# dariopagliaricci/Metal-PathTracer-arm64

Measured on AMD Instinct MI355X. Metric: Msamples/sec (whole node) at 1920×1080, depth 8; PFM RMSE vs Embree ref, higher is better.
Workload: dtype f32; 1 GPU; BASELINE configs[1]: Cornell box + one 70,688-triangle OBJ mesh, 1920x1080, depth 8, 256 spp, seed 1337; partition=8-row bands round-robin over 1 rank(s), RCCL gather of the HDR buffer

## Files before the change

metal-pathtracer-arm64_amd/csrc/kernels/traverse.h:

```cpp
#pragma once

#include "device_types.h"
#include "vec.h"

namespace ptrk {

struct TraceCounters {
    uint32_t nodes;
    uint32_t prims;
    uint32_t waveNodeSteps = 0, wavePrimSteps = 0, leaves = 0;
};

typedef __attribute__((address_space(3))) uint32_t LdsWord;

struct LaneStack {
    LdsWord* lds;
    uint32_t* spill;
    uint32_t spillStride;
    uint32_t limit;
    uint32_t sp;
    __device__ __forceinline__ uint32_t* spillSlot(uint32_t level) const {
        const uint32_t column = blockIdx.x * kTraceBlock + threadIdx.x;
        return spill + static_cast<size_t>(level - kLdsStackLevels) * spillStride + column;
    }
    __device__ __forceinline__ void push(uint32_t v) {
        if (sp < kLdsStackLevels) {
            lds[sp * kTraceBlock] = v;
        } else if (sp < limit) {
            *spillSlot(sp) = v;
        } else {
            return;
        }
        ++sp;
    }
    __device__ __forceinline__ uint32_t pop() {
        --sp;
        return (sp < kLdsStackLevels) ? lds[sp * kTraceBlock] : *spillSlot(sp);
    }
};

typedef uint32_t u32x4 __attribute__((ext_vector_type(4)));

struct SceneMem {
    __amdgpu_buffer_rsrc_t nodes;
    __amdgpu_buffer_rsrc_t tris;
    __amdgpu_buffer_rsrc_t wide;
};

__device__ __forceinline__ SceneMem sceneMem(const SceneView& sc) {
    SceneMem m;
    const void* nodes = sc.useQuantized ? static_cast<const void*>(sc.qnodes) : static_cast<const void*>(sc.nodes);
    m.nodes = __builtin_amdgcn_make_buffer_rsrc(const_cast<void*>(nodes), 0, sc.nodeBytes, 0x00020000);
    m.tris = __builtin_amdgcn_make_buffer_rsrc(const_cast<float4*>(sc.tris), 0, sc.triBytes, 0x00020000);
    m.wide = __builtin_amdgcn_make_buffer_rsrc(const_cast<uint4*>(sc.wnodes), 0, sc.wideBytes, 0x00020000);
    return m;
}

__device__ __forceinline__ uint4 load16u(__amdgpu_buffer_rsrc_t r, uint32_t byteOffset) {
    const u32x4 v = __builtin_amdgcn_raw_buffer_load_b128(r, byteOffset, 0, 0);
    return make_uint4(v.x, v.y, v.z, v.w);
}
__device__ __forceinline__ float4 load16f(__amdgpu_buffer_rsrc_t r, uint32_t byteOffset) {
    const u32x4 v = __builtin_amdgcn_raw_buffer_load_b128(r, byteOffset, 0, 0);
    return make_float4(__uint_as_float(v.x), __uint_as_float(v.y), __uint_as_float(v.z), __uint_as_float(v.w));
}

struct TraceHit {
    float t;
    uint32_t prim;
};

typedef float v2f __attribute__((ext_vector_type(2)));

__device__ __forceinline__ bool slabTest(f3 lo, f3 hi, f3 oi, f3 inv, float tnear, float tfar, float& entry) {
    const v2f tx = __builtin_elementwise_fma((v2f){lo.x, hi.x}, (v2f){inv.x, inv.x}, (v2f){-oi.x, -oi.x});
    const v2f ty = __builtin_elementwise_fma((v2f){lo.y, hi.y}, (v2f){inv.y, inv.y}, (v2f){-oi.y, -oi.y});
    const v2f tz = __builtin_elementwise_fma((v2f){lo.z, hi.z}, (v2f){inv.z, inv.z}, (v2f){-oi.z, -oi.z});
    const float ax = tx.x, bx = tx.y, ay = ty.x, by = ty.y, az = tz.x, bz = tz.y;
    const float t0 = fmaxf(fmaxf(fminf(ax, bx), fminf(ay, by)), fmaxf(fminf(az, bz), tnear));
    const float t1 = fminf(fminf(fmaxf(ax, bx), fmaxf(ay, by)), fminf(fmaxf(az, bz), tfar));
    entry = t0;
    return t0 <= t1 * 1.0000004f;
}

__device__ __forceinline__ bool slabTestOrdered(f3 nearQ, f3 farQ, f3 oi, f3 inv, float tnear, float tfar, float& entry) {
    const v2f tx = __builtin_elementwise_fma((v2f){nearQ.x, farQ.x}, (v2f){inv.x, inv.x}, (v2f){-oi.x, -oi.x});
    const v2f ty = __builtin_elementwise_fma((v2f){nearQ.y, farQ.y}, (v2f){inv.y, inv.y}, (v2f){-oi.y, -oi.y});
    const v2f tz = __builtin_elementwise_fma((v2f){nearQ.z, farQ.z}, (v2f){inv.z, inv.z}, (v2f){-oi.z, -oi.z});
    const float t0 = fmaxf(fmaxf(tx.x, ty.x), fmaxf(tz.x, tnear));
    const float t1 = fminf(fminf(tx.y, ty.y), fminf(tz.y, tfar));
    entry = t0;
    return t0 <= t1 * 1.0000004f;
}

__device__ __forceinline__ bool triangleTest(f3 v0, f3 e1, f3 e2, f3 org, f3 dir, float tnear, float tfar,
                                             float& t, float& u, float& v) {
    const f3 Ng = cross(e2, e1);
    const f3 C = v0 - org;
    const f3 R = cross(C, dir);
    const float den = dot(Ng, dir);
    const float absDen = fabsf(den);
    const float sgn = signbit(den) ? -1.0f : 1.0f;
    const float U = dot(R, e2) * sgn;
    const float V = dot(R, e1) * sgn;
    if (!(den != 0.0f && U >= 0.0f && V >= 0.0f && (U + V) <= absDen)) return false;
    const float T = dot(Ng, C) * sgn;
    if (!(absDen * tnear < T && T <= absDen * tfar)) return false;
    const float rcpAbsDen = 1.0f / absDen;
    t = T * rcpAbsDen;
    u = U * rcpAbsDen;
    v = V * rcpAbsDen;
    return true;
}

__device__ __forceinline__ void triangleUv(f3 v0, f3 e1, f3 e2, f3 org, f3 dir, float& u, float& v) {
    const f3 Ng = cross(e2, e1);
    const f3 C = v0 - org;
    const f3 R = cross(C, dir);
    const float den = dot(Ng, dir);
    const float absDen = fabsf(den);
    const float sgn = signbit(den) ? -1.0f : 1.0f;
    const float U = dot(R, e2) * sgn;
    const float V = dot(R, e1) * sgn;
    const float rcpAbsDen = 1.0f / absDen;
    u = U * rcpAbsDen;
    v = V * rcpAbsDen;
}

__device__ __forceinline__ bool sphereTest(float4 s, f3 org, f3 dir, float tnear, float tfar, float& t) {
    const float rd2 = 1.0f / dot(dir, dir);
    const f3 c0 = mk3(s) - org;
    const float projC0 = dot(c0, dir) * rd2;
    const f3 perp = c0 - projC0 * dir;
    const float l2 = dot(perp, perp);
    const float r2 = s.w * s.w;
    if (!(l2 <= r2)) return false;
    const float td = sqrtf((r2 - l2) * rd2);
    const float tFront = projC0 - td;
    const float tBack = projC0 + td;
    const bool validFront = (tnear <= tFront) && (tFront <= tfar);
    const bool validBack = (tnear <= tBack) && (tBack <= tfar);
    if (!validFront && !validBack) return false;
    t = validFront ? tFront : tBack;
    return true;
}

struct Trav {
    f3 org, dir, inv;
    f3 oi;
    uint32_t selX, selY, selZ;
    float tnear;
    TraceHit hit;
    uint32_t cur;
    uint32_t leafPos;
    bool anyHit;
};

template <int NODES = -1>
__device__ __forceinline__ bool travBegin(const SceneView& sc, Trav& t, f3 org, f3 dir, float tnear, float tfar, bool anyHit,
                                          LaneStack& stack) {
    t.org = org;
    t.dir = dir;
    constexpr float kInvMax = 1.0e28f;
    t.inv = mk3(fminf(fmaxf(__builtin_amdgcn_rcpf(dir.x), -kInvMax), kInvMax), fminf(fmaxf(__builtin_amdgcn_rcpf(dir.y), -kInvMax), kInvMax),
                fminf(fmaxf(__builtin_amdgcn_rcpf(dir.z), -kInvMax), kInvMax));
    if (NODES >= 1 || (NODES < 0 && sc.useQuantized)) {
        const f3 cell = mk3(sc.gridCell[0], sc.gridCell[1], sc.gridCell[2]);
        const f3 invCell = mk3(sc.gridInvCell[0], sc.gridInvCell[1], sc.gridInvCell[2]);
        const f3 orgQ = (org - mk3(sc.gridOrigin[0], sc.gridOrigin[1], sc.gridOrigin[2])) * invCell;
        t.inv = t.inv * cell;
        t.oi = orgQ * t.inv;
    } else {
        t.oi = org * t.inv;
    }
    t.selX = t.inv.x < 0.0f ? 0x01000706u : 0x07060100u;
    t.selY = t.inv.y < 0.0f ? 0x03020504u : 0x05040302u;
    t.selZ = t.inv.z < 0.0f ? 0x01000706u : 0x07060100u;
    t.tnear = tnear;
    t.hit.t = tfar;
    t.hit.prim = kHitMiss;
    t.anyHit = anyHit;
    t.cur = sc.rootRef;
    t.leafPos = 0u;
    stack.sp = 0;
    if (sc.oversizeRef != kRefEmpty) {
        if (sc.rootRef != kRefEmpty) stack.push(sc.rootRef);
        t.cur = sc.oversizeRef;
        return true;
    }
    return sc.rootRef != kRefEmpty;
}

__device__ __forceinline__ bool travAtLeaf(const Trav& t) { return (t.cur & kRefLeafBit) != 0u; }
__device__ __forceinline__ bool travPop(Trav& t, LaneStack& stack) {
    if (stack.sp == 0) return false;
    t.cur = stack.pop();
    t.leafPos = 0u;
    return true;
}

__device__ __forceinline__ f3 gridLo(uint32_t w0, uint32_t w1) {
    return mk3(static_cast<float>(w0 & 0xFFFFu), static_cast<float>(w0 >> 16), static_cast<float>(w1 & 0xFFFFu));
}
__device__ __forceinline__ f3 gridHi(uint32_t w1, uint32_t w2) {
    return mk3(static_cast<float>(w1 >> 16), static_cast<float>(w2 & 0xFFFFu), static_cast<float>(w2 >> 16));
}

template <bool COUNT>
__device__ __forceinline__ bool travWideStep(const SceneMem& mem, Trav& t, LaneStack& stack, TraceCounters& cnt) {
    const uint32_t at = t.cur * 64u;
    const uint4 c0 = load16u(mem.wide, at), c1 = load16u(mem.wide, at + 16u), c2 = load16u(mem.wide, at + 32u), c3 = load16u(mem.wide, at + 48u);
    float k0, k1, k2, k3;
    auto boxTest = [&](const uint4& c, float& k) {
        const uint32_t wx = __builtin_amdgcn_perm(c.y, c.x, t.selX), wy = __builtin_amdgcn_perm(c.z, c.x, t.selY), wz = __builtin_amdgcn_perm(c.z, c.y, t.selZ);
        const f3 nearQ = mk3(static_cast<float>(wx & 0xFFFFu), static_cast<float>(wy & 0xFFFFu), static_cast<float>(wz & 0xFFFFu));
        const f3 farQ = mk3(static_cast<float>(wx >> 16), static_cast<float>(wy >> 16), static_cast<float>(wz >> 16));
        return slabTestOrdered(nearQ, farQ, t.oi, t.inv, t.tnear, t.hit.t, k);
    };
    const bool h0 = boxTest(c0, k0), h1 = boxTest(c1, k1), h2 = boxTest(c2, k2), h3 = boxTest(c3, k3);
    k0 = h0 ? k0 : INFINITY;
    k1 = h1 ? k1 : INFINITY;
    k2 = h2 ? k2 : INFINITY;
    k3 = h3 ? k3 : INFINITY;
    uint32_t r0 = c0.w, r1 = c1.w, r2 = c2.w, r3 = c3.w;
    if (COUNT) ++cnt.nodes;
    t.leafPos = 0u;
    auto exchange = [](float& ka, uint32_t& ra, float& kb, uint32_t& rb) {
        const bool swap = kb < ka;
        const float kLo = swap ? kb : ka, kHi = swap ? ka : kb;
        const uint32_t rLo = swap ? rb : ra, rHi = swap ? ra : rb;
        ka = kLo;
        kb = kHi;
        ra = rLo;
        rb = rHi;
    };
    exchange(k0, r0, k1, r1);
    exchange(k2, r2, k3, r3);
    exchange(k0, r0, k2, r2);
    exchange(k1, r1, k3, r3);
    exchange(k1, r1, k2, r2);
    if (k3 < INFINITY) stack.push(r3);
    if (k2 < INFINITY) stack.push(r2);
    if (k1 < INFINITY) stack.push(r1);
    if (k0 < INFINITY) {
        t.cur = r0;
        return true;
    }
    return travPop(t, stack);
}

template <bool COUNT, int NODES = -1>
__device__ __forceinline__ bool travNodeStep(const SceneView& sc, const SceneMem& mem, Trav& t, LaneStack& stack, TraceCounters& cnt) {
    if (NODES == 2) return travWideStep<COUNT>(mem, t, stack, cnt);
    uint32_t ref0, ref1;
    float e0, e1;
    bool h0, h1;
    if (NODES == 1 || (NODES < 0 && sc.useQuantized)) {
        const uint4 q0 = load16u(mem.nodes, t.cur * 32u), q1 = load16u(mem.nodes, t.cur * 32u + 16u);
        ref0 = q0.w;
        ref1 = q1.w;
        h0 = slabTest(gridLo(q0.x, q0.y), gridHi(q0.y, q0.z), t.oi, t.inv, t.tnear, t.hit.t, e0);
        h1 = slabTest(gridLo(q1.x, q1.y), gridHi(q1.y, q1.z), t.oi, t.inv, t.tnear, t.hit.t, e1);
    } else {
        const uint32_t at = t.cur * 64u;
        const float4 n0 = load16f(mem.nodes, at), n1 = load16f(mem.nodes, at + 16u), n2 = load16f(mem.nodes, at + 32u),
                     n3 = load16f(mem.nodes, at + 48u);
        ref0 = __float_as_uint(n0.w);
        ref1 = __float_as_uint(n1.w);
        h0 = slabTest(mk3(n0), mk3(n1), t.oi, t.inv, t.tnear, t.hit.t, e0);
        h1 = slabTest(mk3(n2), mk3(n3), t.oi, t.inv, t.tnear, t.hit.t, e1);
    }
    h0 = h0 & (ref0 != kRefEmpty);
    h1 = h1 & (ref1 != kRefEmpty);
    if (COUNT) ++cnt.nodes;
    const bool firstIs0 = e0 <= e1;
    const uint32_t nearRef = (h0 & (firstIs0 | !h1)) ? ref0 : ref1;
    const uint32_t farRef = firstIs0 ? ref1 : ref0;
    t.leafPos = 0u;
    if (h0 & h1) stack.push(farRef);
    if (h0 | h1) {
        t.cur = nearRef;
        return true;
    }
    return travPop(t, stack);
}

template <bool COUNT>
__device__ __forceinline__ bool travPrimStep(const SceneView& sc, const SceneMem& mem, Trav& t, LaneStack& stack, TraceCounters& cnt) {
    const uint32_t cur = t.cur;
    const uint32_t first = cur & kRefOffsetMask;
    const uint32_t count = ((cur >> kRefCountShift) & 0xFu) + 1u;
    const uint32_t index = first + t.leafPos;
    if (COUNT) { ++cnt.prims; if (t.leafPos == 0u) { ++cnt.nodes; ++cnt.leaves; } }
    if (cur & kRefSphereBit) {
        float tt;
        if (sphereTest(sc.spheres[index], t.org, t.dir, t.tnear, t.hit.t, tt)) {
            t.hit.t = tt;
            t.hit.prim = index | kHitSphereBit;
            if (t.anyHit) return false;
        }
    } else {
        const uint32_t at = index * 48u;
        const float4 a = load16f(mem.tris, at), b = load16f(mem.tris, at + 16u), c = load16f(mem.tris, at + 32u);
        float tt, u, v;
        if (triangleTest(mk3(a), mk3(b), mk3(c), t.org, t.dir, t.tnear, t.hit.t, tt, u, v) && !(t.anyHit && __float_as_uint(b.w) == t.hit.prim)) {
            t.hit.t = tt;
            t.hit.prim = index;
            if (t.anyHit) return false;
        }
    }
    if (++t.leafPos < count) return true;
    return travPop(t, stack);
}

#ifndef PTR_EXTRA_NODE_STEPS
#define PTR_EXTRA_NODE_STEPS 3
#endif
#ifndef PTR_EXTRA_PRIM_STEPS
#define PTR_EXTRA_PRIM_STEPS 1
#endif
#ifndef PTR_PRIM_BIAS
#define PTR_PRIM_BIAS 2
#endif
#ifndef PTR_REPEAT_NUM
#define PTR_REPEAT_NUM 1
#define PTR_REPEAT_DEN 2
#endif

template <bool COUNT, int NODES = -1>
__device__ __forceinline__ bool travVote(const SceneView& sc, const SceneMem& mem, Trav& t, bool active, LaneStack& stack,
                                         TraceCounters& cnt) {
    const bool wantsPrim = active && travAtLeaf(t);
    const bool wantsNode = active && !travAtLeaf(t);
    const int nPrim = __popcll(__ballot(wantsPrim));
    const int nNode = __popcll(__ballot(wantsNode));
    bool more = true;
    if (nNode >= nPrim * PTR_PRIM_BIAS) {
        if (COUNT) ++cnt.waveNodeSteps;
// ... 38 lines not shown
```

metal-pathtracer-arm64_amd/csrc/kernels/wavefront.hip:

```cpp
#include <hip/hip_runtime.h>

#include <algorithm>

#include "bsdf.h"
#include "device_types.h"
#include "launch.h"
#include <type_traits>
#include "traverse.h"
#include "texture.h"
#include "vec.h"

namespace ptrk {

namespace {

constexpr float kEps = 1.0e-4f;
constexpr float kSpecNeePdfFloor = 1.0e-4f;
constexpr float kSpecNeeInvPdfClamp = 1.0e4f;
constexpr float kMisMin = 1.0e-4f;
constexpr float kMisMax = 0.9999f;
#ifndef PTR_SHADE_BLOCK
#define PTR_SHADE_BLOCK 128
#endif
constexpr uint32_t kShadeBlock = PTR_SHADE_BLOCK;
// ... 308 lines not shown
        const uint32_t idx = prim & ~kHitSphereBit;
        const float4 sp = sc.spheres[idx];
        const uint2 info = sc.sphereInfo[idx];
        const f3 n = normalize(s.position - mk3(sp));
        s.normal = n;
        s.hitShadingNormal = n;
        s.frontFace = dot(dir, n) < 0.0f;
        s.twoSided = true;
        s.primType = 1u;
        s.geomIndex = 0u;
        s.primIndex = info.x;
        s.material = info.y;
        return s;
    }
    const uint32_t triOffset = prim * 48u;
    const float4* tp = byteOffset(sc.tris, triOffset);
    const float4* np = byteOffset(sc.triNormals, triOffset);
    const float4 a = tp[0], b = tp[1], c = tp[2];
    const float4 n0 = np[0], n1 = np[1], n2 = np[2];
    asm volatile("" ::"v"(a.x), "v"(b.x), "v"(c.x), "v"(n0.x), "v"(n1.x), "v"(n2.x));
    const f3 ng = cross(mk3(c), mk3(b));
    if (dot(ng, ng) > 0.0f) s.normal = normalize(ng);
    s.frontFace = dot(dir, s.normal) < 0.0f;
    const f3 adjusted = s.frontFace ? s.normal : -s.normal;
    f3 shading = adjusted;
    const uint32_t meta = __float_as_uint(b.w);
    s.material = __float_as_uint(a.w);
    s.geomIndex = 0u;
    if ((meta >> 30) == 0u) {
        s.primType = 0u;
        s.primIndex = __float_as_uint(c.w);
        s.geomIndex = meta & kTriGeomMask;
        float u, v;
        triangleUv(mk3(a), mk3(b), mk3(c), org, dir, u, v);
        s.bu = u;
        s.bv = v;
        const float w = 1.0f - u - v;
        const f3 interp = (w * mk3(n0) + u * mk3(n1)) + v * mk3(n2);
        if (dot(interp, interp) > 0.0f) {
            shading = normalize(interp);
            if (dot(shading, adjusted) < 0.0f) shading = -shading;
        }
    } else {
        s.primType = 2u;
        s.primIndex = meta & kTriGeomMask;
        shading = mk3(n0);
        if (dot(shading, adjusted) < 0.0f) shading = -shading;
        s.twoSided = __float_as_uint(sc.rects[static_cast<size_t>(s.primIndex) * 5u + 4u].y) != 0u;
    }
    s.hitShadingNormal = shading;
    return s;
}

struct OffsetFrame {
    f3 position, n;
    float distance;
};
__device__ __forceinline__ OffsetFrame offsetFrame(const Surface& s) {
    OffsetFrame of;
    f3 n = s.hitShadingNormal;
    if (dot(n, n) <= 0.0f) n = s.normal;
    if (dot(n, n) <= 0.0f) n = mk3(0.0f, 1.0f, 0.0f);
    of.n = normalize(n);
    of.distance = smax(fabsf(s.t) * 1.0e-4f, kEps);
    of.position = s.position;
    return of;
}
// ... 28 lines not shown
    if (distSq <= 0.0f) return 0.0f;
    const float distance = sqrtf(distSq);
    const f3 direction = toLight / distance;
    float cosLight = dot(-direction, mk3(r[3]));
    if (__float_as_uint(r[4].y) != 0u) {
        cosLight = fabsf(cosLight);
    } else if (cosLight <= 0.0f) {
        return 0.0f;
    }
    if (cosLight <= 0.0f) return 0.0f;
    const float pdfArea = 1.0f / area;
    const float pdfDir = pdfArea * distSq / smax(cosLight, 1.0e-6f);
    return pdfDir * (1.0f / static_cast<float>(sc.rectLightCount));
}

__device__ __forceinline__ bool rectLightHit(const SceneView& sc, const Surface& s, f3 origin, float emissionScale, f3& emission, float& pdf) {
    if (sc.rectLightCount == 0u || sc.rectCount == 0u) return false;
    if (s.primType != 2u || s.primIndex >= sc.rectCount) return false;
    const int32_t li = sc.lightIndexByRect[s.primIndex];
    if (li < 0) return false;
    const float4* L = sc.rectLights + static_cast<size_t>(li) * kRectLightVec4;
    const bool twoSided = L[1].w != 0.0f;
    if (!s.frontFace && !twoSided) return false;
    emission = mk3(L[4]) * emissionScale;
    if (!(dot(emission, emission) > 0.0f)) return false;
    pdf = rectLightPdfForHit(sc, s.primType, s.primIndex, s.position, origin);
    return (pdf > 0.0f) && isfinite(pdf);
}


__device__ __forceinline__ bool nearestRectLight(const SceneView& sc, f3 org, f3 dir, float& tHit, uint32_t& light, uint32_t& half) {
    float best = INFINITY;
    bool found = false;
    for (uint32_t li = 0; li < sc.rectLightCount; ++li) {
        const float4* T = sc.rectLights + static_cast<size_t>(li) * kRectLightVec4 + 5u;
#pragma unroll
        for (uint32_t h = 0; h < 2u; ++h) {
            float tt, tu, tv;
            if (triangleTest(mk3(T[h * 3u]), mk3(T[h * 3u + 1u]), mk3(T[h * 3u + 2u]), org, dir, kEps, best, tt, tu, tv)) {
                best = tt;
                light = li;
                half = h;
                found = true;
            }
        }
    }
    tHit = best;
    return found;
}

__device__ __forceinline__ Surface rectLightSurface(const SceneView& sc, f3 org, f3 dir, float t, uint32_t light, uint32_t half, uint32_t& metaWord) {
    const float4* T = sc.rectLights + static_cast<size_t>(light) * kRectLightVec4 + 5u + half * 3u;
    const float4 b = T[1], c = T[2];
    Surface s;
    s.t = t;
    s.prim = 0u;
    s.bu = 0.0f;
    s.bv = 0.0f;
    s.position = org + t * dir;
    s.normal = mk3(0.0f, 1.0f, 0.0f);
    const f3 ng = cross(mk3(c), mk3(b));
    if (dot(ng, ng) > 0.0f) s.normal = normalize(ng);
    s.hitShadingNormal = s.normal;
    s.frontFace = dot(dir, s.normal) < 0.0f;
    s.twoSided = false;
    metaWord = __float_as_uint(b.w);
    s.primType = 2u;
    s.primIndex = metaWord & kTriGeomMask;
    s.geomIndex = 0u;
    s.material = 0u;
    return s;
}
// ... 61 lines not shown
    if constexpr (COUNT) {
        addCounter(counters, kCntShadowRays, raysAny);
        addCounter(counters, kCntShadowNodes, any.nodes);
        addCounter(counters, kCntShadowPrims, any.prims);
        addCounter(counters, kCntExtendRays, raysClosest);
        addCounter(counters, kCntExtendNodes, closest.nodes);
        addCounter(counters, kCntExtendPrims, closest.prims);
    }
}

}

__global__ void __launch_bounds__(256) k_generate(RenderParams rp, PathPool pool) {
    const uint32_t slot = blockIdx.x * blockDim.x + threadIdx.x;
    if (slot >= pool.slots) return;
    uint32_t flags = 0u, rng = 0u;
    f3 o = mk3(0.0f), d = mk3(0.0f);
    if (slot < rp.itemCount && rp.maxDepth > 0u) {
        beginItem(rp, pool, slot, rng, o, d);
        flags = kFlagAlive | kFlagLastDelta;
    }
    pool.ray0[slot] = mk4(o, d.x);
    pool.ray1[slot] = make_float4(d.y, d.z, 1.0f, __uint_as_float(flags));
    pool.thr[slot] = make_float4(1.0f, 1.0f, 1.0f, __uint_as_float(rng));
    pool.accum[slot] = make_float4(0.0f, 0.0f, 0.0f, __uint_as_float(slot));
    if (pool.signature) pool.signature[slot] = 0u;
    if (pool.cone) pool.cone[slot] = primaryCone(rp);
}

#ifndef PTR_TRAV_WAVES
#define PTR_TRAV_WAVES 8
#endif
#define PTR_EXTEND_ATTR __attribute__((amdgpu_waves_per_eu(PTR_TRAV_WAVES, PTR_TRAV_WAVES)))
template <bool COUNT, bool ALIVE, int NODES>
__global__ void __launch_bounds__(kTraceBlock) PTR_EXTEND_ATTR k_extend(SceneView sc, PathPool pool, uint32_t* spill, uint32_t spillStride, uint32_t* workCounter,
                                                         int kRefillBelow, uint32_t feederChunk, uint32_t* aliveOut) {
    __shared__ uint32_t ldsStack[kLdsStackLevels * kTraceBlock];
    LaneStack stack = laneStack(ldsStack, spill, spillStride, sc);
    TraceCounters cnt{0u, 0u};
    uint32_t rays = 0u;
    uint32_t aliveSeen = 0u;
    uint32_t refills = 0u;
    uint32_t refillCycles = 0u;
    uint32_t activeLanes = 0u, leafLanes = 0u, voteIterations = 0u;
    const long long kernelStart = COUNT ? clock64() : 0ll;

    SceneMem mem = sceneMem(sc);
    bool listed = ALIVE && pool.busyIn != nullptr;
    SubLists lists{0u, pool.slots};
    if (listed) {
        lists.init(pool.busyCountIn, pool.connectRegion);
        if (static_cast<uint64_t>(lists.total) * PTR_BUSY_EXTEND_DIV >= pool.slots) {
            listed = false;
            lists.total = pool.slots;
        }
    }
    WaveFeeder feeder;
    const uint32_t listChunk = shortListChunk(lists.total, (gridDim.x * blockDim.x) >> 6);
    feeder.init(workCounter, lists.total, listed ? listChunk : feederChunk);
    Trav t;
    t.cur = 0u;
    bool active = false;
    uint32_t mySlot = 0u;
    while (true) {
        const int nActive = __popcll(__ballot(active));
        if (nActive < kRefillBelow && !feeder.exhausted) {
            if (COUNT) ++refills;
            const long long refillStart = COUNT ? clock64() : 0ll;
            uint32_t idx = feeder.take(!active);
            if (listed) {
                const uint32_t entry = pool.busyIn[lists.position(idx != WaveFeeder::kNone ? idx : 0u, pool.connectRegion)];
                if (idx != WaveFeeder::kNone) idx = (entry & kBusyAliveBit) ? (entry & ~kBusyAliveBit) : WaveFeeder::kNone;
            }
            const uint32_t at = idx != WaveFeeder::kNone ? idx : 0u;
            const float4 r0 = pool.ray0[at], r1 = pool.ray1[at];
            const bool live = idx != WaveFeeder::kNone && (__float_as_uint(r1.w) & kFlagAlive);
            if (ALIVE) aliveSeen += static_cast<uint32_t>(__popcll(__ballot(live)));
            if (live) {
                mySlot = idx;
                if (COUNT) ++rays;
                active = travBegin<NODES>(sc, t, mk3(r0), mk3(r0.w, r1.x, r1.y), kEps, INFINITY, false, stack);
                if (!active) pool.hit[idx] = make_float2(INFINITY, __uint_as_float(kHitMiss));
            }
            if (COUNT) {
                asm volatile("" ::"v"(t.inv.x), "v"(t.oi.x));
                refillCycles += static_cast<uint32_t>(clock64() - refillStart);
            }
            continue;
        }
        if (nActive == 0) break;
        if (COUNT) {
            activeLanes += static_cast<uint32_t>(nActive);
            leafLanes += static_cast<uint32_t>(__popcll(__ballot(active && travAtLeaf(t))));
            ++voteIterations;
        }
        if (!travVote<COUNT, NODES>(sc, mem, t, active, stack, cnt)) {
            active = false;
            pool.hit[mySlot] = make_float2(t.hit.t, __uint_as_float(t.hit.prim));
        }
    }
    if (ALIVE) {
        if (laneId() == 0 && aliveSeen != 0u) atomicAdd(aliveOut, aliveSeen);
    }
    if (COUNT) {
        addCounter(pool.counters, kCntExtendRays, rays);
        addCounter(pool.counters, kCntExtendNodes, cnt.nodes);
        addCounter(pool.counters, kCntExtendPrims, cnt.prims);
        addCounter(pool.counters, kCntExtendLeaves, cnt.leaves);
        addCounter(pool.counters, kCntExtendWaveNodeSteps, cnt.waveNodeSteps);
        addCounter(pool.counters, kCntExtendWavePrimSteps, cnt.wavePrimSteps);
        addCounter(pool.counters, kCntExtendRefillPasses, refills);
        addCounter(pool.counters, kCntExtendActiveLanes, activeLanes >> 6);
        addCounter(pool.counters, kCntExtendLeafLanes, leafLanes >> 6);
        addCounter(pool.counters, kCntExtendVoteIterations, voteIterations);
        addCounter(pool.counters, kCntExtendRefillTicks, refillCycles >> 4);
        addCounter(pool.counters, kCntExtendWaveTicks, static_cast<uint32_t>((clock64() - kernelStart) >> 4));
    }
}
// ... 379 lines not shown
    const UniformRows Lu = uniformRows(sc.rectLights);
    auto row = [&](uint32_t i) { return ONE ? Lu[i] : Lv[i]; };
    const float4 l0 = row(0), l1 = row(1), l2 = row(2), l3 = row(3);
    const f3 samplePoint = (mk3(l0) + lu * mk3(l1)) + lv * mk3(l2);
    const f3 toLight = samplePoint - sf.position;
    const float distSq = dot(toLight, toLight);
    if (!(distSq > 0.0f && l0.w > 0.0f)) return false;
    const float distance = sqrtf(distSq);
    const f3 ldir = toLight / distance;
    float cosLight = dot(-ldir, mk3(l3));
    if (l1.w != 0.0f) cosLight = fabsf(cosLight);
    if (!(cosLight > 0.0f)) return false;
    const float pdfArea = 1.0f / l0.w;
    const float pdfDir = pdfArea * distSq / smax(cosLight, 1.0e-6f);
    const float pdf = pdfDir * (1.0f / static_cast<float>(nL));
    const f3 emission = mk3(row(4)) * rp.emissionScale;
    const float nDotL = smax(dot(n, ldir), 0.0f);
    if (!(pdf > 0.0f && isfinite(pdf) && (dot(emission, emission) > 0.0f) && nDotL > 0.0f)) return false;
    if (COUNT) counts.stage[4] += 1u;
    const BsdfEvalResult be = evalBsdf<SSS, MATS>(mat, sf.position, n, wo, ldir, cc);
    if (!neeContributes<SSS>(be, cc)) return false;
    const float w = neeWeight<SSS>(pdf, be.pdf, cc);
    f3 contrib = (emission * be.value) * nDotL;
    contrib *= w / pdf;
    if (!finite3(contrib)) return false;
    const f3 clamped = clampFirefly(thr, contrib, cc);
    if (!(clamped.x > 0.0f || clamped.y > 0.0f || clamped.z > 0.0f)) return false;
    const float shadowMax = smax(distance * (1.0f - rp.shadowSlack) - kEps, kEps);
    const f3 shadowOrg = offsetOrigin(of, ldir);
    float tt, tu, tv;
    bool occludedByLight = false;
    if (COUNT) counts.stage[5] += 1u;
    if (l3.w != 0.0f) {
        occludedByLight = triangleTest(mk3(row(5)), mk3(row(6)), mk3(row(7)), shadowOrg, ldir, kEps, shadowMax, tt, tu, tv) ||
                          triangleTest(mk3(row(8)), mk3(row(9)), mk3(row(10)), shadowOrg, ldir, kEps, shadowMax, tt, tu, tv);
    }
    if (occludedByLight) return false;
    if (COUNT) counts.stage[6] += 1u;
    storeRecord(pool, slot, 0u, 0u, shadowOrg, shadowMax, ldir, clamped, static_cast<float>(depth), mk3(0.0f));
    return true;
}

template <bool SSS>
__device__ __forceinline__ bool surfaceIsDelta(const Mat& mat, uint32_t type, const ClampCfg& cc) {
    bool surfaceDelta = materialIsDelta(mat);
    if (SSS && cc.metalPbr && type == 7u) surfaceDelta = mat.roughness01() <= 1.0e-3f;
    return surfaceDelta;
}

constexpr int kShadeDense = 0, kShadeListed = 1, kShadeTail = 2;
template <bool COUNT, bool SSS, bool TEX, int MODE, uint32_t MATS = kAllMaterials>
__device__ __forceinline__ void shadeSlot(const RenderParams& rp, const SceneView& sc, const PathPool& pool, const uint32_t slot, const bool inRange,
                                          const bool drained, const uint32_t listWave, ShadeCounts& counts, const EnvLodView& env) {
    constexpr bool TAIL = MODE == kShadeTail;
    const long long tLoad = partBegin<COUNT>();
    const uint32_t at = inRange ? slot : 0u;
    float4 ray1v = pool.ray1[at];
    if (!TAIL && drained) {
        const uint32_t peek = __float_as_uint(ray1v.w);
        const bool busy = inRange && (peek & (kFlagAlive | kFlagFlush | (kFlagPendingMask << kFlagPendingShift))) != 0u;
        if (__ballot(busy) == 0ull) return;
    }
    const float4 ray0v = pool.ray0[at];
    uint2 reservation = make_uint2(0u, 0u);
    if (MODE == kShadeDense && (slot & ~63u) < pool.slots) reservation = pool.itemReserve[__builtin_amdgcn_readfirstlane(slot / 64u)];
    const float2 hitv = pool.hit[at];
    const float4 thr4 = pool.thr[at];
    const float4 acc4 = pool.accum[at];
// ... 590 lines not shown
    f3 result = mk3(0.0f);
    if (COUNT) ++raysClosest;
    const TraceHit h = traverse<false, COUNT>(sc, org, dir, kEps, INFINITY, stack, cntClosest);
    if (h.prim == kHitMiss || sc.materialCount == 0u) return result;
    const Surface cs = reconstruct(sc, org, dir, h.t, h.prim);
    f3 tmpE;
    float tmpP;
    if (sc.rectLightCount > 0u && rectLightHit(sc, cs, org, rp.emissionScale, tmpE, tmpP)) return result;
    const Mat cm{sc.materials + static_cast<size_t>(min(cs.material, sc.materialCount - 1u)) * kMaterialVec4};
    if (!materialIsDelta(cm)) return result;
    f3 cn = cs.normal;
    if (dot(cn, cn) <= 0.0f) cn = mk3(0.0f, 1.0f, 0.0f);
    cn = normalize(cn);
    const f3 cin = normalize(dir);
    const BsdfSampleResult s2 = sampleBsdf(cm, cs.position, cn, -cin, cin, cs.frontFace, rngCopy, cc);
    if (!(s2.pdf > 0.0f && s2.isDelta && dot(s2.dir, s2.dir) > 0.0f && finite3(s2.weight))) return result;
    const f3 d2 = normalize(s2.dir);
    const f3 o2 = offsetOrigin(cs, d2);
    const f3 w2 = weight * s2.weight;
    const float pdf2 = bsdfPdf * s2.pdf;
    if (sc.envSampling) {
        if (COUNT) ++raysAny;
        result += alongEnv<COUNT>(rp, sc, cc, o2, d2, w2, pdf2, thr, stack, cntAny);
    }
    if (sc.rectLightCount > 0u) {
        if (COUNT) ++raysClosest;
        result += alongRect<COUNT>(rp, sc, cc, o2, d2, w2, pdf2, thr, stack, cntClosest);
    }
    return result;
}

}

template <bool COUNT, int NODES>
__global__ void __launch_bounds__(kTraceBlock) PTR_EXTEND_ATTR k_connect(RenderParams rp, SceneView sc, PathPool pool, uint32_t* spill, uint32_t spillStride,
                                                          uint32_t* workCounter, int kRefillBelow, uint32_t feederChunk) {
    __shared__ uint32_t ldsStack[kLdsStackLevels * kTraceBlock];
    LaneStack stack = laneStack(ldsStack, spill, spillStride, sc);
    TraceCounters cnt{0u, 0u}, cntClosest{0u, 0u};
    uint32_t rays = 0u, raysClosest = 0u, early = 0u;
    const ClampCfg cc = clampCfg(rp);

    SceneMem mem = sceneMem(sc);
    SubLists lists;
    lists.init(pool.connectCount, pool.connectRegion);
    WaveFeeder feeder;
    feeder.init(workCounter, lists.total, shortListChunk(lists.total, (gridDim.x * blockDim.x) >> 6));
    Trav t;
    t.cur = 0u;
    bool active = false;
    uint32_t mySlot = 0u, bits = 0u;
    float4* const recBase = pool.rec[0].org;
    const uint32_t slots = pool.recStride;
    uint32_t myRecAt = 0u;
    while (true) {
        const int nActive = __popcll(__ballot(active));
        const bool idleBits = __ballot(!active && bits != 0u) != 0ull;
        if (nActive < kRefillBelow && (idleBits || !feeder.exhausted)) {
            if (!feeder.exhausted) {
                const uint32_t idx = feeder.take(!active && bits == 0u);
                const uint32_t at = lists.position(idx != WaveFeeder::kNone ? idx : 0u, pool.connectRegion);
                if (idx != WaveFeeder::kNone) {
                    const uint32_t entry = pool.connectList[at];
                    mySlot = entry & ((1u << kConnectMaskShift) - 1u);
                    bits = entry >> kConnectMaskShift;
                }
            }
            if (!active && bits != 0u) {
                const uint32_t rec = static_cast<uint32_t>(__ffs(static_cast<int>(bits))) - 1u;
                bits &= bits - 1u;
                myRecAt = rec * 4u * slots + mySlot;
                const float4 o4 = recBase[myRecAt], d4 = recBase[myRecAt + slots];
                const uint32_t kind = __float_as_uint(d4.w);
                if (kind != 2u) {
                    const bool any = kind != 1u;
                    if (COUNT) { if (any) ++rays; else ++raysClosest; }
                    active = travBegin<NODES>(sc, t, mk3(o4), mk3(d4), kEps, any ? o4.w : INFINITY, any, stack);
                    if (kind == 3u) t.hit.prim = __float_as_uint(recBase[myRecAt + 3u * slots].x);
                    if (!active && kind == 1u) recBase[myRecAt + 2u * slots] = make_float4(0.0f, 0.0f, 0.0f, 0.0f);
                }
            }
            continue;
        }
        if (nActive == 0) break;
        {
            TraceCounters step{0u, 0u};
            const bool more = travVote<COUNT, NODES>(sc, mem, t, active, stack, step);
            if (COUNT) {
                TraceCounters& dst = t.anyHit ? cnt : cntClosest;
                dst.nodes += step.nodes;
                dst.prims += step.prims;
            }
            if (!more) {
                active = false;
                float4* const a = recBase + myRecAt + 2u * slots;
                if (t.anyHit) {
                    if (COUNT) early += anyHitFound(t.hit.prim) ? 1u : 0u;
                    if (anyHitFound(t.hit.prim)) *a = make_float4(0.0f, 0.0f, 0.0f, 0.0f);
                } else {
                    const float4 a4 = *a;
                    const f3 c = rectContribution(rp, sc, cc, t.org, t.dir, t.hit, mk3(a4), a4.w, mk3(recBase[myRecAt + 3u * slots]));
                    *a = mk4(c, 0.0f);
                }
            }
        }
    }
    addTraceCounters<COUNT>(pool.counters, rays, cnt, raysClosest, cntClosest);
    if (COUNT) addCounter(pool.counters, kCntShadowEarlyExit, early);
}

template <bool COUNT>
__global__ void __launch_bounds__(kTraceBlock) k_connect_chain(RenderParams rp, SceneView sc, PathPool pool, uint32_t* spill, uint32_t spillStride) {
    __shared__ uint32_t ldsStack[kLdsStackLevels * kTraceBlock];
    const uint32_t gtid = blockIdx.x * kTraceBlock + threadIdx.x;
    LaneStack stack = laneStack(ldsStack, spill, spillStride, sc);
    TraceCounters cnt{0u, 0u}, cntClosest{0u, 0u};
    uint32_t rays = 0u, raysClosest = 0u;
    const ClampCfg cc = clampCfg(rp);
    for (uint32_t slot = gtid; slot < pool.slots; slot += gridDim.x * kTraceBlock) {
        if (!((__float_as_uint(pool.ray1[slot].w) >> kFlagPendingShift) & (1u << 4))) continue;
        const ShadowRecordView& r = pool.rec[4];
        const float4 d4 = r.dir[slot];
        if (__float_as_uint(d4.w) != 2u) continue;
        const float4 o4 = r.org[slot], a4 = r.a[slot];
        const f3 c = mneeChain<COUNT>(rp, sc, cc, mk3(o4), mk3(d4), __float_as_uint(o4.w), mk3(a4), a4.w, mk3(r.b[slot]), stack, cnt,
                                      cntClosest, rays, raysClosest);
        r.a[slot] = mk4(c, 0.0f);
    }
    addTraceCounters<COUNT>(pool.counters, rays, cnt, raysClosest, cntClosest);
}

__global__ void __launch_bounds__(256) k_tail_collect(PathPool pool, uint32_t* list, uint32_t* listCount) {
    __shared__ uint32_t found[4][64];
    const uint32_t wave = threadIdx.x >> 6, lane = laneId();
// ... 156 lines not shown
            f3 sn = sf.hitShadingNormal;
            if (dot(sn, sn) <= 0.0f) sn = sf.normal;
            if (mat.type() == 2u) sn = sf.normal;
            sn = normalize(sn);
            a = mk4(mat.baseColor(), 1.0f);
            n = mk4(sn * 0.5f + mk3(0.5f), h.t);
        }
        albedo[pixel] = a;
        normal[pixel] = n;
    }
}

__device__ __forceinline__ PtrHit ptrHitOf(const SceneView& sc, f3 org, f3 dir, const TraceHit& h, bool anyHit) {
    float hu = 0.0f, hv = 0.0f;
    PtrHit r;
    r.t = -1.0f;
    r.u = 0.0f;
    r.v = 0.0f;
    r.primType = 0u;
    r.geomIndex = 0u;
    r.primIndex = 0u;
    r.ng[0] = r.ng[1] = r.ng[2] = 0.0f;
    r.pad = 0u;
    if (h.prim != kHitMiss) {
        r.t = anyHit ? 0.0f : h.t;
        if (!anyHit) {
            if (h.prim & kHitSphereBit) {
                r.primType = 1u;
                r.primIndex = sc.sphereInfo[h.prim & kHitIndexMask].x;
            } else {
                const float4* tp = sc.tris + static_cast<size_t>(h.prim & kHitIndexMask) * 3u;
                const float4 t0 = tp[0], t1 = tp[1], t2 = tp[2];
                const uint32_t meta = __float_as_uint(t1.w);
                triangleUv(mk3(t0), mk3(t1), mk3(t2), org, dir, hu, hv);
                r.u = hu;
                r.v = hv;
                const f3 ng = cross(mk3(t2), mk3(t1));
                r.ng[0] = ng.x;
                r.ng[1] = ng.y;
                r.ng[2] = ng.z;
                if ((meta >> 30) == 0u) {
                    r.primType = 0u;
                    r.geomIndex = meta & kTriGeomMask;
                    r.primIndex = __float_as_uint(t2.w);
                } else {
                    r.primType = 2u;
                    r.primIndex = meta & kTriGeomMask;
                }
            }
        }
    }
    return r;
}

template <bool ANY>
__global__ void __launch_bounds__(kTraceBlock) k_trace_rays(SceneView sc, const float4* rays, uint64_t n, PtrHit* out, uint32_t* spill,
                                                             uint32_t spillStride, uint64_t* counters) {
    __shared__ uint32_t ldsStack[kLdsStackLevels * kTraceBlock];
    const uint32_t gtid = blockIdx.x * kTraceBlock + threadIdx.x;
    LaneStack stack = laneStack(ldsStack, spill, spillStride, sc);
    TraceCounters cnt{0u, 0u};
    for (uint64_t i = gtid; i < n; i += static_cast<uint64_t>(gridDim.x) * kTraceBlock) {
        const float4 a = rays[i * 2u], b = rays[i * 2u + 1u];
        const f3 org = mk3(a), dir = mk3(b);
        const TraceHit h = traverse<ANY, true>(sc, org, dir, a.w, b.w, stack, cnt);
        out[i] = ptrHitOf(sc, org, dir, h, ANY);
    }
// ... 488 lines not shown
```

Before: 2529 Msamples/s.

## Pack ray/triangle math into paired f32 ops and reload cold kernel args

Rewrites the triangle test and slab test so the ray and triangle data are held as float pairs, letting the compiler use packed v_pk_* f32 FMA/add/mul and inline-asm cross blends. The ray state now stores origin/direction pairs and precomputed (inv, -oi) slab pairs instead of separate org/dir/inv/oi vectors. Cold scene and render params in k_extend and k_connect are re-read from the kernarg segment through an opaque pointer, so they are not kept live in registers across the traversal loop. The aim is fewer VALU instructions and lower register pressure in the traversal kernels. In exchange it relies on inline asm and compiler behaviour, and could change rounding slightly.

```diff
diff --git a/metal-pathtracer-arm64_amd/csrc/kernels/traverse.h b/metal-pathtracer-arm64_amd/csrc/kernels/traverse.h
--- a/metal-pathtracer-arm64_amd/csrc/kernels/traverse.h
+++ b/metal-pathtracer-arm64_amd/csrc/kernels/traverse.h
@@ -40,6 +40,7 @@
 };
 
 typedef uint32_t u32x4 __attribute__((ext_vector_type(4)));
+typedef float v4f __attribute__((ext_vector_type(4)));
 
 struct SceneMem {
     __amdgpu_buffer_rsrc_t nodes;
@@ -60,6 +61,9 @@
     const u32x4 v = __builtin_amdgcn_raw_buffer_load_b128(r, byteOffset, 0, 0);
     return make_uint4(v.x, v.y, v.z, v.w);
 }
+__device__ __forceinline__ v4f load16v(__amdgpu_buffer_rsrc_t r, uint32_t byteOffset) {
+    return __builtin_bit_cast(v4f, __builtin_amdgcn_raw_buffer_load_b128(r, byteOffset, 0, 0));
+}
 __device__ __forceinline__ float4 load16f(__amdgpu_buffer_rsrc_t r, uint32_t byteOffset) {
     const u32x4 v = __builtin_amdgcn_raw_buffer_load_b128(r, byteOffset, 0, 0);
     return make_float4(__uint_as_float(v.x), __uint_as_float(v.y), __uint_as_float(v.z), __uint_as_float(v.w));
@@ -72,39 +76,123 @@
 
 typedef float v2f __attribute__((ext_vector_type(2)));
 
-__device__ __forceinline__ bool slabTest(f3 lo, f3 hi, f3 oi, f3 inv, float tnear, float tfar, float& entry) {
-    const v2f tx = __builtin_elementwise_fma((v2f){lo.x, hi.x}, (v2f){inv.x, inv.x}, (v2f){-oi.x, -oi.x});
-    const v2f ty = __builtin_elementwise_fma((v2f){lo.y, hi.y}, (v2f){inv.y, inv.y}, (v2f){-oi.y, -oi.y});
-    const v2f tz = __builtin_elementwise_fma((v2f){lo.z, hi.z}, (v2f){inv.z, inv.z}, (v2f){-oi.z, -oi.z});
+struct SlabAxes {
+    v2f x, y, z;
+};
+
+__device__ __forceinline__ v2f slabPlanes(float p0, float p1, v2f axis) {
+    return __builtin_elementwise_fma((v2f){p0, p1}, __builtin_shufflevector(axis, axis, 0, 0), __builtin_shufflevector(axis, axis, 1, 1));
+}
+
+__device__ __forceinline__ float minWithTfar(float a, float tfar) {
+    float r;
+    asm("v_min_f32 %0, %1, %2" : "=v"(r) : "v"(a), "v"(tfar));
+    return r;
+}
+
+__device__ __forceinline__ bool slabTest(f3 lo, f3 hi, const SlabAxes& ax3, float tnear, float tfar, float& entry) {
+    const v2f tx = slabPlanes(lo.x, hi.x, ax3.x), ty = slabPlanes(lo.y, hi.y, ax3.y), tz = slabPlanes(lo.z, hi.z, ax3.z);
     const float ax = tx.x, bx = tx.y, ay = ty.x, by = ty.y, az = tz.x, bz = tz.y;
     const float t0 = fmaxf(fmaxf(fminf(ax, bx), fminf(ay, by)), fmaxf(fminf(az, bz), tnear));
-    const float t1 = fminf(fminf(fmaxf(ax, bx), fmaxf(ay, by)), fminf(fmaxf(az, bz), tfar));
+    const float t1 = fminf(fminf(fmaxf(ax, bx), fmaxf(ay, by)), minWithTfar(fmaxf(az, bz), tfar));
     entry = t0;
     return t0 <= t1 * 1.0000004f;
 }
 
-__device__ __forceinline__ bool slabTestOrdered(f3 nearQ, f3 farQ, f3 oi, f3 inv, float tnear, float tfar, float& entry) {
-    const v2f tx = __builtin_elementwise_fma((v2f){nearQ.x, farQ.x}, (v2f){inv.x, inv.x}, (v2f){-oi.x, -oi.x});
-    const v2f ty = __builtin_elementwise_fma((v2f){nearQ.y, farQ.y}, (v2f){inv.y, inv.y}, (v2f){-oi.y, -oi.y});
-    const v2f tz = __builtin_elementwise_fma((v2f){nearQ.z, farQ.z}, (v2f){inv.z, inv.z}, (v2f){-oi.z, -oi.z});
+__device__ __forceinline__ bool slabTestOrdered(f3 nearQ, f3 farQ, const SlabAxes& ax3, float tnear, float tfar, float& entry) {
+    const v2f tx = slabPlanes(nearQ.x, farQ.x, ax3.x), ty = slabPlanes(nearQ.y, farQ.y, ax3.y), tz = slabPlanes(nearQ.z, farQ.z, ax3.z);
     const float t0 = fmaxf(fmaxf(tx.x, ty.x), fmaxf(tz.x, tnear));
-    const float t1 = fminf(fminf(tx.y, ty.y), fminf(tz.y, tfar));
+    const float t1 = fminf(fminf(tx.y, ty.y), minWithTfar(tz.y, tfar));
     entry = t0;
     return t0 <= t1 * 1.0000004f;
 }
 
-__device__ __forceinline__ bool triangleTest(f3 v0, f3 e1, f3 e2, f3 org, f3 dir, float tnear, float tfar,
-                                             float& t, float& u, float& v) {
-    const f3 Ng = cross(e2, e1);
-    const f3 C = v0 - org;
-    const f3 R = cross(C, dir);
-    const float den = dot(Ng, dir);
-    const float absDen = fabsf(den);
-    const float sgn = signbit(den) ? -1.0f : 1.0f;
-    const float U = dot(R, e2) * sgn;
-    const float V = dot(R, e1) * sgn;
-    if (!(den != 0.0f && U >= 0.0f && V >= 0.0f && (U + V) <= absDen)) return false;
-    const float T = dot(Ng, C) * sgn;
+struct s2f {
+    float x, y;
+};
+__device__ __forceinline__ s2f operator*(s2f a, s2f b) { return s2f{a.x * b.x, a.y * b.y}; }
+__device__ __forceinline__ s2f operator-(s2f a, s2f b) { return s2f{a.x - b.x, a.y - b.y}; }
+
+template <int LO, int HI> __device__ __forceinline__ v2f pick(v2f p) { return __builtin_shufflevector(p, p, LO, HI); }
+template <int LO, int HI> __device__ __forceinline__ s2f pick(s2f p) { return s2f{LO ? p.y : p.x, HI ? p.y : p.x}; }
+__device__ __forceinline__ v2f crossBlend(v2f m1, v2f m2) {
+    v2f xy;
+    asm("v_pk_add_f32 %0, %1, %2 neg_lo:[0,1] neg_hi:[1,0]" : "=v"(xy) : "v"(m1), "v"(m2));
+    return xy;
+}
+__device__ __forceinline__ s2f crossBlend(s2f m1, s2f m2) { return s2f{m1.x - m2.x, m2.y - m1.y}; }
+__device__ __forceinline__ float sumHalves(v2f p) {
+    float r;
+    asm("v_add_f32 %0, %1, %2" : "=v"(r) : "v"(p.x), "v"(p.y));
+    return r;
+}
+__device__ __forceinline__ float sumHalves(s2f p) { return p.x + p.y; }
+
+template <typename P>
+struct RayPairsT {
+    P orgXY, dirXY, orgZdirZ;
+};
+typedef RayPairsT<v2f> RayPairs;
+template <typename P = v2f>
+__device__ __forceinline__ RayPairsT<P> rayPairs(f3 org, f3 dir) { return RayPairsT<P>{P{org.x, org.y}, P{dir.x, dir.y}, P{org.z, dir.z}}; }
+__device__ __forceinline__ f3 rayOrg(const RayPairs& r) { return mk3(r.orgXY.x, r.orgXY.y, r.orgZdirZ.x); }
+__device__ __forceinline__ f3 rayDir(const RayPairs& r) { return mk3(r.dirXY.x, r.dirXY.y, r.orgZdirZ.y); }
+
+template <typename P>
+struct TrianglePairsT {
+    P v0XY, v0Z_, e1XY, e1Z_, e2XY, e2Z_;
+};
+__device__ __forceinline__ TrianglePairsT<v2f> trianglePairs(v4f a, v4f b, v4f c) { return TrianglePairsT<v2f>{a.xy, a.zw, b.xy, b.zw, c.xy, c.zw}; }
+__device__ __forceinline__ TrianglePairsT<v2f> trianglePairs(const float4& a, const float4& b, const float4& c) {
+    return TrianglePairsT<v2f>{(v2f){a.x, a.y}, (v2f){a.z, a.w}, (v2f){b.x, b.y}, (v2f){b.z, b.w}, (v2f){c.x, c.y}, (v2f){c.z, c.w}};
+}
+__device__ __forceinline__ TrianglePairsT<s2f> triangleScalars(const float4& a, const float4& b, const float4& c) {
+    return TrianglePairsT<s2f>{s2f{a.x, a.y}, s2f{a.z, a.z}, s2f{b.x, b.y}, s2f{b.z, b.z}, s2f{c.x, c.y}, s2f{c.z, c.z}};
+}
+
+template <int AZ, int BZ, typename P>
+__device__ __forceinline__ P crossPairs(P aXY, P aZ_, P bXY, P bZ_, float& z) {
+    const P bYX = pick<1, 0>(bXY);
+    const P m1 = pick<1, 0>(aXY) * pick<BZ, BZ>(bZ_);
+    const P m2 = pick<AZ, AZ>(aZ_) * bYX;
+    const P m3 = aXY * bYX;
+    z = m3.x - m3.y;
+    return crossBlend(m1, m2);
+}
+template <typename P>
+__device__ __forceinline__ float dotPairs(P aXY, float aZ, P bXY, float bZ) {
+    const P m = aXY * bXY;
+    return (m.x + m.y) + aZ * bZ;
+}
+
+template <typename P>
+struct TriangleTermsT {
+    P ngXY, cXY, uv;
+    float ngZ, cZ, den, sgn;
+};
+template <typename P>
+__device__ __forceinline__ TriangleTermsT<P> triangleTerms(const TrianglePairsT<P>& tri, const RayPairsT<P>& ray) {
+    TriangleTermsT<P> k;
+    float rZ;
+    k.ngXY = crossPairs<0, 0>(tri.e2XY, tri.e2Z_, tri.e1XY, tri.e1Z_, k.ngZ);
+    k.cXY = tri.v0XY - ray.orgXY;
+    const P cZ_ = tri.v0Z_ - ray.orgZdirZ;
+    k.cZ = cZ_.x;
+    const float dirZ = ray.orgZdirZ.y;
+    const P rXY = crossPairs<0, 1>(k.cXY, cZ_, ray.dirXY, ray.orgZdirZ, rZ);
+    k.den = dotPairs(k.ngXY, k.ngZ, ray.dirXY, dirZ);
+    k.sgn = signbit(k.den) ? -1.0f : 1.0f;
+    k.uv = P{dotPairs(rXY, rZ, tri.e2XY, tri.e2Z_.x), dotPairs(rXY, rZ, tri.e1XY, tri.e1Z_.x)} * P{k.sgn, k.sgn};
+    return k;
+}
+
+template <typename P>
+__device__ __forceinline__ bool triangleTest(const TrianglePairsT<P>& tri, const RayPairsT<P>& ray, float tnear, float tfar, float& t, float& u, float& v) {
+    const TriangleTermsT<P> k = triangleTerms(tri, ray);
+    const float absDen = fabsf(k.den);
+    const float U = k.uv.x, V = k.uv.y;
+    if (!(k.den != 0.0f && U >= 0.0f && V >= 0.0f && sumHalves(k.uv) <= absDen)) return false;
+    const float T = dotPairs(k.ngXY, k.ngZ, k.cXY, k.cZ) * k.sgn;
     if (!(absDen * tnear < T && T <= absDen * tfar)) return false;
     const float rcpAbsDen = 1.0f / absDen;
     t = T * rcpAbsDen;
@@ -113,18 +201,12 @@
     return true;
 }
 
-__device__ __forceinline__ void triangleUv(f3 v0, f3 e1, f3 e2, f3 org, f3 dir, float& u, float& v) {
-    const f3 Ng = cross(e2, e1);
-    const f3 C = v0 - org;
-    const f3 R = cross(C, dir);
-    const float den = dot(Ng, dir);
-    const float absDen = fabsf(den);
-    const float sgn = signbit(den) ? -1.0f : 1.0f;
-    const float U = dot(R, e2) * sgn;
-    const float V = dot(R, e1) * sgn;
-    const float rcpAbsDen = 1.0f / absDen;
-    u = U * rcpAbsDen;
-    v = V * rcpAbsDen;
+template <typename P>
+__device__ __forceinline__ void triangleUv(const TrianglePairsT<P>& tri, const RayPairsT<P>& ray, float& u, float& v) {
+    const TriangleTermsT<P> k = triangleTerms(tri, ray);
+    const float rcpAbsDen = 1.0f / fabsf(k.den);
+    u = k.uv.x * rcpAbsDen;
+    v = k.uv.y * rcpAbsDen;
 }
 
 __device__ __forceinline__ bool sphereTest(float4 s, f3 org, f3 dir, float tnear, float tfar, float& t) {
@@ -146,8 +228,8 @@
 }
 
 struct Trav {
-    f3 org, dir, inv;
-    f3 oi;
+    RayPairs ray;
+    SlabAxes slab;
     uint32_t selX, selY, selZ;
     float tnear;
     TraceHit hit;
@@ -159,23 +241,24 @@
 template <int NODES = -1>
 __device__ __forceinline__ bool travBegin(const SceneView& sc, Trav& t, f3 org, f3 dir, float tnear, float tfar, bool anyHit,
                                           LaneStack& stack) {
-    t.org = org;
-    t.dir = dir;
+    t.ray = rayPairs(org, dir);
     constexpr float kInvMax = 1.0e28f;
-    t.inv = mk3(fminf(fmaxf(__builtin_amdgcn_rcpf(dir.x), -kInvMax), kInvMax), fminf(fmaxf(__builtin_amdgcn_rcpf(dir.y), -kInvMax), kInvMax),
-                fminf(fmaxf(__builtin_amdgcn_rcpf(dir.z), -kInvMax), kInvMax));
+    f3 inv = mk3(fminf(fmaxf(__builtin_amdgcn_rcpf(dir.x), -kInvMax), kInvMax), fminf(fmaxf(__builtin_amdgcn_rcpf(dir.y), -kInvMax), kInvMax),
+                 fminf(fmaxf(__builtin_amdgcn_rcpf(dir.z), -kInvMax), kInvMax));
+    f3 oi;
     if (NODES >= 1 || (NODES < 0 && sc.useQuantized)) {
         const f3 cell = mk3(sc.gridCell[0], sc.gridCell[1], sc.gridCell[2]);
         const f3 invCell = mk3(sc.gridInvCell[0], sc.gridInvCell[1], sc.gridInvCell[2]);
         const f3 orgQ = (org - mk3(sc.gridOrigin[0], sc.gridOrigin[1], sc.gridOrigin[2])) * invCell;
-        t.inv = t.inv * cell;
-        t.oi = orgQ * t.inv;
+        inv = inv * cell;
+        oi = orgQ * inv;
     } else {
-        t.oi = org * t.inv;
-    }
-    t.selX = t.inv.x < 0.0f ? 0x01000706u : 0x07060100u;
-    t.selY = t.inv.y < 0.0f ? 0x03020504u : 0x05040302u;
-    t.selZ = t.inv.z < 0.0f ? 0x01000706u : 0x07060100u;
+        oi = org * inv;
+    }
+    t.slab = SlabAxes{(v2f){inv.x, -oi.x}, (v2f){inv.y, -oi.y}, (v2f){inv.z, -oi.z}};
+    t.selX = inv.x < 0.0f ? 0x01000706u : 0x07060100u;
+    t.selY = inv.y < 0.0f ? 0x03020504u : 0x05040302u;
+    t.selZ = inv.z < 0.0f ? 0x01000706u : 0x07060100u;
     t.tnear = tnear;
     t.hit.t = tfar;
     t.hit.prim = kHitMiss;
@@ -215,7 +298,7 @@
         const uint32_t wx = __builtin_amdgcn_perm(c.y, c.x, t.selX), wy = __builtin_amdgcn_perm(c.z, c.x, t.selY), wz = __builtin_amdgcn_perm(c.z, c.y, t.selZ);
         const f3 nearQ = mk3(static_cast<float>(wx & 0xFFFFu), static_cast<float>(wy & 0xFFFFu), static_cast<float>(wz & 0xFFFFu));
         const f3 farQ = mk3(static_cast<float>(wx >> 16), static_cast<float>(wy >> 16), static_cast<float>(wz >> 16));
-        return slabTestOrdered(nearQ, farQ, t.oi, t.inv, t.tnear, t.hit.t, k);
+        return slabTestOrdered(nearQ, farQ, t.slab, t.tnear, t.hit.t, k);
     };
     const bool h0 = boxTest(c0, k0), h1 = boxTest(c1, k1), h2 = boxTest(c2, k2), h3 = boxTest(c3, k3);
     k0 = h0 ? k0 : INFINITY;
@@ -259,16 +342,16 @@
         const uint4 q0 = load16u(mem.nodes, t.cur * 32u), q1 = load16u(mem.nodes, t.cur * 32u + 16u);
         ref0 = q0.w;
         ref1 = q1.w;
-        h0 = slabTest(gridLo(q0.x, q0.y), gridHi(q0.y, q0.z), t.oi, t.inv, t.tnear, t.hit.t, e0);
-        h1 = slabTest(gridLo(q1.x, q1.y), gridHi(q1.y, q1.z), t.oi, t.inv, t.tnear, t.hit.t, e1);
+        h0 = slabTest(gridLo(q0.x, q0.y), gridHi(q0.y, q0.z), t.slab, t.tnear, t.hit.t, e0);
+        h1 = slabTest(gridLo(q1.x, q1.y), gridHi(q1.y, q1.z), t.slab, t.tnear, t.hit.t, e1);
     } else {
         const uint32_t at = t.cur * 64u;
         const float4 n0 = load16f(mem.nodes, at), n1 = load16f(mem.nodes, at + 16u), n2 = load16f(mem.nodes, at + 32u),
                      n3 = load16f(mem.nodes, at + 48u);
         ref0 = __float_as_uint(n0.w);
         ref1 = __float_as_uint(n1.w);
-        h0 = slabTest(mk3(n0), mk3(n1), t.oi, t.inv, t.tnear, t.hit.t, e0);
-        h1 = slabTest(mk3(n2), mk3(n3), t.oi, t.inv, t.tnear, t.hit.t, e1);
+        h0 = slabTest(mk3(n0), mk3(n1), t.slab, t.tnear, t.hit.t, e0);
+        h1 = slabTest(mk3(n2), mk3(n3), t.slab, t.tnear, t.hit.t, e1);
     }
     h0 = h0 & (ref0 != kRefEmpty);
     h1 = h1 & (ref1 != kRefEmpty);
@@ -294,16 +377,18 @@
     if (COUNT) { ++cnt.prims; if (t.leafPos == 0u) { ++cnt.nodes; ++cnt.leaves; } }
     if (cur & kRefSphereBit) {
         float tt;
-        if (sphereTest(sc.spheres[index], t.org, t.dir, t.tnear, t.hit.t, tt)) {
+        if (sphereTest(sc.spheres[index], rayOrg(t.ray), rayDir(t.ray), t.tnear, t.hit.t, tt)) {
             t.hit.t = tt;
             t.hit.prim = index | kHitSphereBit;
             if (t.anyHit) return false;
         }
     } else {
         const uint32_t at = index * 48u;
-        const float4 a = load16f(mem.tris, at), b = load16f(mem.tris, at + 16u), c = load16f(mem.tris, at + 32u);
+        const v4f a = load16v(mem.tris, at);
+        v4f b = load16v(mem.tris, at + 16u), c = load16v(mem.tris, at + 32u);
+        asm("" : "+v"(b), "+v"(c));
         float tt, u, v;
-        if (triangleTest(mk3(a), mk3(b), mk3(c), t.org, t.dir, t.tnear, t.hit.t, tt, u, v) && !(t.anyHit && __float_as_uint(b.w) == t.hit.prim)) {
+        if (triangleTest(trianglePairs(a, b, c), t.ray, t.tnear, t.hit.t, tt, u, v) && !(t.anyHit && __float_as_uint(b.w) == t.hit.prim)) {
             t.hit.t = tt;
             t.hit.prim = index;
             if (t.anyHit) return false;
diff --git a/metal-pathtracer-arm64_amd/csrc/kernels/wavefront.hip b/metal-pathtracer-arm64_amd/csrc/kernels/wavefront.hip
--- a/metal-pathtracer-arm64_amd/csrc/kernels/wavefront.hip
+++ b/metal-pathtracer-arm64_amd/csrc/kernels/wavefront.hip
@@ -364,7 +364,7 @@
         s.primIndex = __float_as_uint(c.w);
         s.geomIndex = meta & kTriGeomMask;
         float u, v;
-        triangleUv(mk3(a), mk3(b), mk3(c), org, dir, u, v);
+        triangleUv(triangleScalars(a, b, c), rayPairs<s2f>(org, dir), u, v);
         s.bu = u;
         s.bv = v;
         const float w = 1.0f - u - v;
@@ -459,12 +459,13 @@
 __device__ __forceinline__ bool nearestRectLight(const SceneView& sc, f3 org, f3 dir, float& tHit, uint32_t& light, uint32_t& half) {
     float best = INFINITY;
     bool found = false;
+    const RayPairsT<s2f> ray = rayPairs<s2f>(org, dir);
     for (uint32_t li = 0; li < sc.rectLightCount; ++li) {
         const float4* T = sc.rectLights + static_cast<size_t>(li) * kRectLightVec4 + 5u;
 #pragma unroll
         for (uint32_t h = 0; h < 2u; ++h) {
             float tt, tu, tv;
-            if (triangleTest(mk3(T[h * 3u]), mk3(T[h * 3u + 1u]), mk3(T[h * 3u + 2u]), org, dir, kEps, best, tt, tu, tv)) {
+            if (triangleTest(triangleScalars(T[h * 3u], T[h * 3u + 1u], T[h * 3u + 2u]), ray, kEps, best, tt, tu, tv)) {
                 best = tt;
                 light = li;
                 half = h;
@@ -592,6 +593,12 @@
 #define PTR_TRAV_WAVES 8
 #endif
 #define PTR_EXTEND_ATTR __attribute__((amdgpu_waves_per_eu(PTR_TRAV_WAVES, PTR_TRAV_WAVES)))
+__device__ __forceinline__ const SceneView* extendColdScene() {
+    auto p = __builtin_amdgcn_kernarg_segment_ptr();
+    asm volatile("" : "+s"(p));
+    return (const SceneView*)p;
+}
+
 template <bool COUNT, bool ALIVE, int NODES>
 __global__ void __launch_bounds__(kTraceBlock) PTR_EXTEND_ATTR k_extend(SceneView sc, PathPool pool, uint32_t* spill, uint32_t spillStride, uint32_t* workCounter,
                                                          int kRefillBelow, uint32_t feederChunk, uint32_t* aliveOut) {
@@ -639,11 +646,11 @@
             if (live) {
                 mySlot = idx;
                 if (COUNT) ++rays;
-                active = travBegin<NODES>(sc, t, mk3(r0), mk3(r0.w, r1.x, r1.y), kEps, INFINITY, false, stack);
+                active = travBegin<NODES>(*extendColdScene(), t, mk3(r0), mk3(r0.w, r1.x, r1.y), kEps, INFINITY, false, stack);
                 if (!active) pool.hit[idx] = make_float2(INFINITY, __uint_as_float(kHitMiss));
             }
             if (COUNT) {
-                asm volatile("" ::"v"(t.inv.x), "v"(t.oi.x));
+                asm volatile("" ::"v"(t.slab.x));
                 refillCycles += static_cast<uint32_t>(clock64() - refillStart);
             }
             continue;
@@ -1089,8 +1096,9 @@
     bool occludedByLight = false;
     if (COUNT) counts.stage[5] += 1u;
     if (l3.w != 0.0f) {
-        occludedByLight = triangleTest(mk3(row(5)), mk3(row(6)), mk3(row(7)), shadowOrg, ldir, kEps, shadowMax, tt, tu, tv) ||
-                          triangleTest(mk3(row(8)), mk3(row(9)), mk3(row(10)), shadowOrg, ldir, kEps, shadowMax, tt, tu, tv);
+        const RayPairsT<s2f> shadowRay = rayPairs<s2f>(shadowOrg, ldir);
+        occludedByLight = triangleTest(triangleScalars(row(5), row(6), row(7)), shadowRay, kEps, shadowMax, tt, tu, tv) ||
+                          triangleTest(triangleScalars(row(8), row(9), row(10)), shadowRay, kEps, shadowMax, tt, tu, tv);
     }
     if (occludedByLight) return false;
     if (COUNT) counts.stage[6] += 1u;
@@ -1747,6 +1755,16 @@
 
 }
 
+struct ConnectColdArgs {
+    RenderParams rp;
+    SceneView sc;
+};
+__device__ __forceinline__ const ConnectColdArgs* connectColdArgs() {
+    auto p = __builtin_amdgcn_kernarg_segment_ptr();
+    asm volatile("" : "+s"(p));
+    return (const ConnectColdArgs*)p;
+}
+
 template <bool COUNT, int NODES>
 __global__ void __launch_bounds__(kTraceBlock) PTR_EXTEND_ATTR k_connect(RenderParams rp, SceneView sc, PathPool pool, uint32_t* spill, uint32_t spillStride,
                                                           uint32_t* workCounter, int kRefillBelow, uint32_t feederChunk) {
@@ -1754,7 +1772,6 @@
     LaneStack stack = laneStack(ldsStack, spill, spillStride, sc);
     TraceCounters cnt{0u, 0u}, cntClosest{0u, 0u};
     uint32_t rays = 0u, raysClosest = 0u, early = 0u;
-    const ClampCfg cc = clampCfg(rp);
 
     SceneMem mem = sceneMem(sc);
     SubLists lists;
@@ -1790,7 +1807,7 @@
                 if (kind != 2u) {
                     const bool any = kind != 1u;
                     if (COUNT) { if (any) ++rays; else ++raysClosest; }
-                    active = travBegin<NODES>(sc, t, mk3(o4), mk3(d4), kEps, any ? o4.w : INFINITY, any, stack);
+                    active = travBegin<NODES>(connectColdArgs()->sc, t, mk3(o4), mk3(d4), kEps, any ? o4.w : INFINITY, any, stack);
                     if (kind == 3u) t.hit.prim = __float_as_uint(recBase[myRecAt + 3u * slots].x);
                     if (!active && kind == 1u) recBase[myRecAt + 2u * slots] = make_float4(0.0f, 0.0f, 0.0f, 0.0f);
                 }
@@ -1814,7 +1831,9 @@
                     if (anyHitFound(t.hit.prim)) *a = make_float4(0.0f, 0.0f, 0.0f, 0.0f);
                 } else {
                     const float4 a4 = *a;
-                    const f3 c = rectContribution(rp, sc, cc, t.org, t.dir, t.hit, mk3(a4), a4.w, mk3(recBase[myRecAt + 3u * slots]));
+                    const ConnectColdArgs* cold = connectColdArgs();
+                    const f3 c = rectContribution(cold->rp, cold->sc, clampCfg(cold->rp), rayOrg(t.ray), rayDir(t.ray), t.hit, mk3(a4), a4.w,
+                                                  mk3(recBase[myRecAt + 3u * slots]));
                     *a = mk4(c, 0.0f);
                 }
             }
@@ -2037,7 +2056,7 @@
                 const float4* tp = sc.tris + static_cast<size_t>(h.prim & kHitIndexMask) * 3u;
                 const float4 t0 = tp[0], t1 = tp[1], t2 = tp[2];
                 const uint32_t meta = __float_as_uint(t1.w);
-                triangleUv(mk3(t0), mk3(t1), mk3(t2), org, dir, hu, hv);
+                triangleUv(trianglePairs(t0, t1, t2), rayPairs(org, dir), hu, hv);
                 r.u = hu;
                 r.v = hv;
                 const f3 ng = cross(mk3(t2), mk3(t1));
```

Measured after the change: 2541 Msamples/s, median of 6. Within noise of the previous version (+0.5%).
